# hadimsnj/SGRACEx1

Measured on AMD Instinct MI355X. Metric: edges aggregated/sec, 2-layer GCN forward, higher is better.
Workload: dtype f16 (f32 accumulate); 1 GPU; s100m; nodes_per_gpu=4194304, edges_per_gpu=104193983, generator=uniform, f_in=1433, hidden=64, layer1=gemm_mode=0 sparse X, relu=1, layer2=gemm_mode=1 dense X, relu=0, exchange=none

## Files before the change

### sgracex1_amd/csrc/layer.hip

```cpp
#include "sgx_internal.h"

namespace {

struct Carve {
    size_t h_off, h_bytes;
    size_t w_off, w_bytes;
    size_t s_off, s_bytes;
    size_t g_off, g_bytes;
    size_t q_off, q_bytes;
    size_t qb, qx, qa, qt;
    size_t qw;
    int64_t ldc;
    size_t total;
};

bool repitch_x(const sgx_layer_desc *d)
{
    return sgx_ldh(d->dtype, d->M_fea) != d->M_fea && (int64_t)d->M_adj * d->M_fea >= (int64_t)1 << 22;
}

bool int8_form(const sgx_layer_desc *d)
{
    if (!d->quant || d->gemm_mode != 1 || d->quant->qbits > 8 || d->P_w > 256) return false;
    if (d->quant->flags & SGX_QUANT_INT8) return true;
    return (d->quant->flags & SGX_QUANT_INT8_AUTO) && d->M_fea > 128;
}

Carve carve(const sgx_layer_desc *d)
{
    Carve c;
    c.qw = 0;
    c.ldc = 0;
    const size_t es = sgx_elem_size(d->dtype);
    const size_t ldh = (size_t)sgx_ldh(d->dtype, d->P_w);
    size_t off = 0;
    if (d->order == SGX_ORDER_AGGREGATE_FIRST) {
        const size_t ldz = (size_t)sgx_ldh(d->dtype, d->M_fea);
        c.h_off = off; c.h_bytes = sgx_align_up((size_t)d->N_adj * ldz * es, 256); off += c.h_bytes;
        c.w_off = off; c.w_bytes = repitch_x(d) ? sgx_align_up((size_t)d->M_adj * ldz * es, 256) : 0; off += c.w_bytes;
        c.s_off = off; c.s_bytes = sgx_spmm_scratch_bytes(d->plan_adj, d->M_fea); off += c.s_bytes;
        c.g_off = off; c.g_bytes = 0;
        c.q_off = off; c.q_bytes = 0; c.qb = c.qx = c.qa = c.qt = 0;
        c.total = off;
        return c;
    }
    c.h_off = off; c.h_bytes = sgx_align_up((size_t)d->M_adj * ldh * es, 256); off += c.h_bytes;
    c.w_off = off; c.w_bytes = d->gemm_mode == 0 ? sgx_align_up((size_t)d->M_fea * ldh * es, 256) : 0; off += c.w_bytes;
    size_t s1 = sgx_spmm_scratch_bytes(d->plan_adj, d->P_w);
    size_t s2 = d->gemm_mode == 0 ? sgx_spmm_scratch_bytes(d->plan_fea, d->P_w) : 0;
    c.s_off = off; c.s_bytes = s1 > s2 ? s1 : s2; off += c.s_bytes;
    c.g_off = off; c.g_bytes = d->gat_mode ? sgx_gat_scratch_bytes(d->M_adj, d->P_w, d->gat_heads, d->gat_fill_dead_rows, d->plan_adj) : 0; off += c.g_bytes;
    c.q_off = off; c.q_bytes = 0; c.qb = c.qx = c.qa = c.qt = 0;
    if (d->quant) {
        const sgx_quant *q = d->quant;
        size_t o = 0;
        if (int8_form(d)) {
            c.ldc = (int64_t)sgx_align_up((size_t)d->M_fea, 16);
            c.qb = o; o += sgx_align_up((size_t)d->P_w * c.ldc, 256);
            c.qx = o; o += sgx_align_up((size_t)d->M_adj * c.ldc, 256);
            c.qw = o; o += sgx_xw_dense_i8_workspace_bytes(d->P_w);
        } else {
            c.qb = o; o += sgx_align_up((size_t)d->P_w * d->M_fea * 4, 256);
            c.qx = o; o += sgx_align_up((d->gemm_mode == 0 ? (size_t)q->nnz_fea : (size_t)d->M_adj * d->M_fea) * 4, 256);
        }
        c.qa = o; o += (q->flags & SGX_QUANT_ADJ_DONE) ? 0 : sgx_align_up((size_t)q->nnz_adj * 4, 256);
        c.qt = o; o += d->gat_mode ? sgx_align_up((size_t)2 * d->P_w * 4, 256) : 0;
        c.q_bytes = o; off += o;
    }
    c.total = off;
    return c;
}

int check_desc(const sgx_layer_desc *d)
{
    if (!d) return SGX_ERR_NULL;
    if (d->N_adj < 0 || d->M_adj < 0 || d->M_fea < 1 || d->P_w < 1) return SGX_ERR_SHAPE;
    if (d->dtype != SGX_F16 && d->dtype != SGX_F32) return SGX_ERR_UNSUPPORTED;
    if (d->gemm_mode != 0 && d->gemm_mode != 1) return SGX_ERR_UNSUPPORTED;
    if (d->order != SGX_ORDER_REFERENCE && d->order != SGX_ORDER_AGGREGATE_FIRST) return SGX_ERR_UNSUPPORTED;
    if (d->order == SGX_ORDER_AGGREGATE_FIRST &&
        (d->gemm_mode != 1 || d->gat_mode || d->quant || d->acc_mode != SGX_ACC_F32))
        return SGX_ERR_UNSUPPORTED;
    if (d->quant) {
        const sgx_quant *q = d->quant;
        if (d->dtype != SGX_F32 || d->acc_mode != SGX_ACC_F32) return SGX_ERR_UNSUPPORTED;
        if (q->qbits < 1 || q->qbits > 16 || q->scale_fea < 0 || q->scale_fea > 30 || q->internal_bits < 1 ||
            q->internal_bits > 30)
            return SGX_ERR_UNSUPPORTED;
        if (q->nnz_adj < 0 || q->nnz_fea < 0) return SGX_ERR_SHAPE;
        if (q->zero_adj != 0.0f || (d->gemm_mode == 0 && q->zero_fea != 0.0f)) return SGX_ERR_UNSUPPORTED;
    }
    return SGX_OK;
}

}

extern "C" size_t sgx_layer_workspace_bytes(const sgx_layer_desc *desc)
{
    if (check_desc(desc) != SGX_OK) return 0;
    return carve(desc).total;
}

extern "C" int sgx_xw_sparse(int dtype, int acc_mode, int spmm_block, int n_rows, int M_fea, int P,
                             const int32_t *rowPtr, const int32_t *columnIndex, const void *values,
                             const void *W_rowmajor, int64_t ldw, void *H, int64_t ldh,
                             const sgx_plan *plan, void *scratch, size_t scratch_bytes, void *stream)
{
    return sgx_spmm_launch(dtype, acc_mode, spmm_block, 0, n_rows, M_fea, P, rowPtr, columnIndex, values,
                           W_rowmajor, ldw, H, ldh, plan, scratch, scratch_bytes, (hipStream_t)stream, nullptr, nullptr, 0,
                           true);
}

namespace {
int thread_count(int32_t t) { return t < 1 ? 1 : t; }

int layer_forward(const sgx_layer_desc *d, const sgx_gat_stats *stats, void *stream)
{
    int rc = check_desc(d);
    if (rc != SGX_OK) return rc;
    if (d->bias_count > 0) return SGX_OK;
    if (d->N_adj == 0) return SGX_OK;
    if (!d->B || !d->D || !d->rowPtr_adj || !d->values_fea) return SGX_ERR_NULL;
    if (d->gemm_mode == 0 && (!d->rowPtr_fea)) return SGX_ERR_NULL;
    const Carve c = carve(d);
    if (!d->workspace || d->workspace_bytes < c.total) return SGX_ERR_WORKSPACE;
    if ((uintptr_t)d->workspace % 256 != 0) return SGX_ERR_ALIGN;

    hipStream_t s = (hipStream_t)stream;
    char *ws = (char *)d->workspace;
    void *H = ws + c.h_off;
    void *W = ws + c.w_off;
    void *scratch = c.s_bytes ? ws + c.s_off : nullptr;
    const int64_t ldh = sgx_ldh(d->dtype, d->P_w);

    if (d->order == SGX_ORDER_AGGREGATE_FIRST) {
        if (!d->values_adj && d->M_adj > 0) return SGX_ERR_NULL;
        const int64_t ldz = sgx_ldh(d->dtype, d->M_fea);
        const void *table = d->values_fea;
        int64_t ld_table = d->M_fea;
        if (c.w_bytes) {
            const size_t es = sgx_elem_size(d->dtype);
            rc = sgx_repitch_rows(d->values_fea, (int64_t)d->M_fea * es, W, ldz * (int64_t)es, (int)(d->M_fea * es), d->M_adj, s);
            if (rc != SGX_OK) return rc;
            table = W;
            ld_table = ldz;
        }
        if (d->ev_agg_begin) SGX_HIP_CHECK(hipEventRecord((hipEvent_t)d->ev_agg_begin, s));
        rc = sgx_spmm_launch(d->dtype, d->acc_mode, 1, 0, d->N_adj, d->M_adj, d->M_fea, d->rowPtr_adj,
                             d->columnIndex_adj, d->values_adj, table, ld_table, H, ldz, d->plan_adj, scratch,
                             c.s_bytes, s, nullptr, nullptr, 0);
        if (rc != SGX_OK) return rc;
        if (d->ev_agg_end) SGX_HIP_CHECK(hipEventRecord((hipEvent_t)d->ev_agg_end, s));
        return sgx_xw_dense_ep(d->dtype, d->acc_mode, 1, d->N_adj, d->M_fea, d->P_w, H, ldz, d->B, d->M_fea, d->D, d->P_w, s,
                               sgx_no_epilogue(), d->relu);
    }

    const void *B = d->B, *values_fea = d->values_fea, *values_adj = d->values_adj, *attention = d->attention;
    const sgx_quant *q = d->quant;
    if (q) {
        if (!d->values_adj) return SGX_ERR_NULL;
        float *qbase = (float *)(ws + c.q_off);
        float *Bq = (float *)((char *)qbase + c.qb), *Xq = (float *)((char *)qbase + c.qx);
        if (c.ldc) {
            rc = sgx_quantize_codes_i8(1, q->qbits, q->inv_scale_w, q->zero_w, d->P_w, d->M_fea, (const float *)d->B, d->M_fea,
                                       (int8_t *)Bq, c.ldc, s);
            if (rc != SGX_OK) return rc;
            rc = sgx_quantize_codes_i8(0, q->qbits, q->inv_scale_fea, q->zero_fea, d->M_adj, d->M_fea, (const float *)d->values_fea,
                                       d->M_fea, (int8_t *)Xq, c.ldc, s);
            if (rc != SGX_OK) return rc;
        } else {
            rc = sgx_fake_quantize(1, q->qbits, q->inv_scale_w, q->zero_w, (int64_t)d->P_w * d->M_fea, (const float *)d->B, Bq, s);
            if (rc != SGX_OK) return rc;
            const int64_t nx = d->gemm_mode == 0 ? q->nnz_fea : (int64_t)d->M_adj * d->M_fea;
            rc = sgx_fake_quantize(0, q->qbits, q->inv_scale_fea, q->zero_fea, nx, (const float *)d->values_fea, Xq, s);
            if (rc != SGX_OK) return rc;
        }
        B = Bq; values_fea = Xq;
        if (!(q->flags & SGX_QUANT_ADJ_DONE)) {
            float *Aq = (float *)((char *)qbase + c.qa);
            rc = sgx_fake_quantize(0, q->qbits, q->inv_scale_adj, q->zero_adj, q->nnz_adj, (const float *)d->values_adj, Aq, s);
            if (rc != SGX_OK) return rc;
            values_adj = Aq;
        }
        if (d->gat_mode) {
            if (!d->attention) return SGX_ERR_NULL;
            float *Tq = (float *)((char *)qbase + c.qt);
            rc = sgx_fake_quantize(1, q->qbits, q->inv_scale_w, q->zero_w, (int64_t)2 * d->P_w, (const float *)d->attention, Tq, s);
            if (rc != SGX_OK) return rc;
            attention = Tq;
        }
    }

    sgx_epilogue ep_h = sgx_no_epilogue(), ep_d = sgx_no_epilogue();
    if (q) {
        ep_h = sgx_requant_epilogue(q->scale_fea, q->internal_bits);
        ep_d.out_scale = q->deq_factor;
    }

    int scores_ready = 0;
    if (d->gat_mode && !q && d->gemm_mode == 1 && d->acc_mode == SGX_ACC_F32 && attention &&
        sgx_gat_scores_fusable(d->dtype, d->P_w, d->gat_heads, d->plan_adj)) {
        const int heads = d->gat_heads < 1 ? 1 : d->gat_heads;
        float *gs = (float *)(ws + c.g_off);
        const sgx_gat_scratch lay = sgx_gat_scratch_layout(d->M_adj, d->P_w, heads, d->gat_fill_dead_rows, d->plan_adj);
        const bool direct = d->P_w / heads == 32;
        float *s1 = gs + (direct ? lay.s1 : lay.sp1), *s2 = gs + (direct ? lay.s2 : lay.sp2);
        rc = (direct || lay.has_partials)
                 ? sgx_xw_dense_scores(d->M_adj, d->M_fea, d->P_w, values_fea, d->M_fea, B, d->M_fea, H, ldh, attention, heads, s1, s2, s)
                 : SGX_ERR_UNSUPPORTED;
        if (rc == SGX_OK && !direct) rc = sgx_gat_scores_combine(gs, lay, d->M_adj, d->P_w, heads, s);
        if (rc == SGX_OK) scores_ready = 1;
// ... 109 lines not shown
```

### sgracex1_amd/csrc/sgx_internal.h

```cpp
#pragma once
#include <hip/hip_runtime.h>
#include <stdint.h>
#include <stddef.h>

#include <type_traits>

#include "sgx.h"

#define SGX_HIP_CHECK(expr)                     \
    do {                                        \
        hipError_t _e = (expr);                 \
        if (_e != hipSuccess) return SGX_ERR_HIP; \
    } while (0)

#define SGX_LAUNCH_CHECK()                                   \
    do {                                                     \
        if (hipGetLastError() != hipSuccess) return SGX_ERR_HIP; \
    } while (0)

typedef _Float16 f16;

struct sgx_tuning {
    bool gat_one_pass, gat_no_fused_scores;
    int gat_fused;
    int gat_scan;
    bool xw_no_wlds, xw_no_stationary_f32, xw_sparse_no_lds, xw_short_tiles, xw_no_lds;
    bool xtg_scalar, xtg_wave_tiles;
    bool spmm_no_short_tail;
    int spmm_cpl;
    int xw_sparse_lpr;
    int xw_sparse_streams;
    int plan_long_threshold;
    int plan_chunk;
    float plan_reorder_below;
};
const sgx_tuning &sgx_tune();

static inline size_t sgx_elem_size(int dtype) { return dtype == SGX_F16 ? 2 : 4; }
static inline size_t sgx_align_up(size_t x, size_t a) { return (x + a - 1) / a * a; }
static inline int sgx_next_pow2(int x) { int p = 1; while (p < x) p <<= 1; return p; }

struct sgx_plan {
    int n_rows;
    int64_t nnz;
    int long_threshold;
    int chunk;
    int n_long;
    int n_tasks;
    int32_t *long_row;
    int32_t *long_first;
    int32_t *task_row;
    int32_t *task_e0;
    int32_t *task_e1;
    int32_t *row_order;
    int n_ordered;
    int n_multi;
    uint8_t *win_order;
    int32_t *scan_win;
    int64_t n_scan_win;
    float natural_utilization;
    int max_degree;
};

static inline int64_t sgx_ldh(int dtype, int P) {
    const int64_t es = dtype == SGX_F16 ? 2 : 4;
    const int64_t row = ((int64_t)P * es + 15) / 16 * 16;
    int64_t pitch = row;
    if (row < 128) {
        pitch = 16;
        while (pitch < row) pitch *= 2;
    } else {
        const int64_t lines = (row + 127) / 128 * 128;
        if (3 * lines <= 4 * row) pitch = lines;
    }
    return pitch / es;
}

struct sgx_epilogue {
    float out_scale, rq_shift, rq_bound, rq_ten_pow;
};
static inline sgx_epilogue sgx_no_epilogue() { return sgx_epilogue{0.0f, 0.0f, 0.0f, 0.0f}; }
sgx_epilogue sgx_requant_epilogue(int scale_fea, int internal_bits);
__device__ __forceinline__ float sgx_requant_value(float v, const sgx_epilogue &ep)
{
#pragma clang fp contract(off)
    v = v * ep.rq_shift;
    v = v < -ep.rq_bound ? -ep.rq_bound : v;
    v = v > ep.rq_bound ? ep.rq_bound : v;
    return rintf(v * ep.rq_ten_pow) / ep.rq_ten_pow;
}

int sgx_refhalf_csr(int spmm_block, int threads, int relu, int n_rows, int n_cols, int n_feat, const int32_t *rowPtr, const int32_t *columnIndex,
                    const void *values, const void *table, int64_t ldt, void *out, int64_t ldo, hipStream_t s);
int sgx_refhalf_dense(int spmm_block, int threads, int n_rows, int M, int n_feat, const void *X, int64_t ldx, const void *Wt,
                      int64_t ldw, void *out, int64_t ldo, hipStream_t s);

int sgx_spmm_launch(int dtype, int acc_mode, int spmm_block, int relu, int n_rows, int n_cols, int n_feat,
                    const int32_t *rowPtr, const int32_t *columnIndex, const void *values,
                    const void *H, int64_t ldh, void *D, int64_t ldd,
                    const sgx_plan *plan, void *scratch, size_t scratch_bytes, hipStream_t stream,
                    const float *acc_in = nullptr, float *acc_out = nullptr, int64_t ld_acc = 0,
                    bool fea_stage = false, int ref_threads = 1, sgx_epilogue ep = sgx_no_epilogue());

bool sgx_spmm_table_big(int dtype, int n_cols, int64_t ldh, int n_feat);

bool sgx_xw_sparse_lds_applicable(int dtype, int n_rows, int m_fea, int n_feat, int64_t ldh, const sgx_plan *plan);
int sgx_xw_sparse_lds(int dtype, int n_rows, int m_fea, int n_feat, const int32_t *rowPtr, const int32_t *columnIndex,
                      const void *values, const void *W, int64_t ldw, void *H, int64_t ldh, const sgx_plan *plan,
                      sgx_epilogue ep, hipStream_t stream);

int sgx_repitch_rows(const void *src, int64_t src_pitch, void *dst, int64_t dst_pitch, int row_bytes, int64_t n_rows,
                     hipStream_t stream);
int sgx_xw_dense_wlds(int n_rows, int M, int P, const void *X, int64_t ldx, const void *Wt, int64_t ldw, void *H, int64_t ldh,
                      int relu, hipStream_t stream);
int sgx_xw_dense_wlds_f32(int n_rows, int M, int P, const void *X, int64_t ldx, const void *Wt, int64_t ldw, void *H, int64_t ldh,
                          int h_aligned, sgx_epilogue ep, int relu, hipStream_t stream);
int sgx_xw_dense_ep(int dtype, int acc_mode, int spmm_block, int n_rows, int M_fea, int P, const void *X, int64_t ldx,
                    const void *Wt, int64_t ldw, void *H, int64_t ldh, hipStream_t stream, sgx_epilogue ep, int relu = 0);
int sgx_gat_aggregate_ep(int dtype, int relu, int fill_dead_rows, int n_rows, int n_cols, int n_feat, int n_heads, float alpha,
                         const int32_t *rowPtr, const int32_t *columnIndex, const void *values, const void *Wh, int64_t ldh,
                         const void *attention, void *D, int64_t ldd, float *E, float *S, const sgx_plan *plan,
                         float *s_scratch, hipStream_t stream, float out_scale, const float *ext_fill = nullptr, int ext_n = 0,
                         int scores_ready = 0);

struct sgx_gat_scratch {
    size_t s1, s2;
    size_t slabs, mean;
    size_t sp1, sp2;
    size_t pacc, pm, pl;
    size_t row_m, row_l;
    size_t weights, dead;
    size_t total;
    int ldp;
    bool has_partials, has_split, has_two_stage;
};
sgx_gat_scratch sgx_gat_scratch_layout(int n_cols, int n_feat, int n_heads, int fill_dead_rows, const sgx_plan *plan);

struct sgx_gat_args {
    int dtype, lpr;
    int relu, n_rows, n_cols, n_feat, n_heads;
    float alpha;
    const int32_t *rowptr, *col;
    const void *val, *Wh, *att;
    int64_t ldh, ldd;
    unsigned h_bytes, ld_bytes;
    void *D;
    float *E, *S;
    float *scratch;
    sgx_gat_scratch lay;
    const float *fill;
    int uniform_n;
    float out_scale;
    const sgx_plan *plan_any;
    const sgx_plan *plan;
    int vec_ok, vec_store;
    int scores_ready;
    hipStream_t stream;
};

template <typename T, int VEC, typename F>
int sgx_gat_dispatch_lpr(int lpr, F &&f)
{
    switch (lpr) {
    case 1: return f(T(), std::integral_constant<int, VEC>(), std::integral_constant<int, 1>());
    case 2: return f(T(), std::integral_constant<int, VEC>(), std::integral_constant<int, 2>());
    case 4: return f(T(), std::integral_constant<int, VEC>(), std::integral_constant<int, 4>());
    case 8: return f(T(), std::integral_constant<int, VEC>(), std::integral_constant<int, 8>());
    case 16: return f(T(), std::integral_constant<int, VEC>(), std::integral_constant<int, 16>());
    case 32: return f(T(), std::integral_constant<int, VEC>(), std::integral_constant<int, 32>());
    default: return f(T(), std::integral_constant<int, VEC>(), std::integral_constant<int, 64>());
    }
}
template <typename F>
int sgx_gat_dispatch(const sgx_gat_args &a, F &&f)
{
    if (a.dtype == SGX_F16) return a.vec_ok ? sgx_gat_dispatch_lpr<f16, 8>(a.lpr, f) : sgx_gat_dispatch_lpr<f16, 1>(a.lpr, f);
    return a.vec_ok ? sgx_gat_dispatch_lpr<float, 4>(a.lpr, f) : sgx_gat_dispatch_lpr<float, 1>(a.lpr, f);
}

int sgx_gat_one_pass(const sgx_gat_args &a);
int sgx_gat_alpha_stage(const sgx_gat_args &a, float *W, bool scan);
int sgx_gat_weighted(const sgx_gat_args &a, const float *W);
int sgx_gat_stats_check(const sgx_gat_stats *st, int n_cols, int n_heads);
int sgx_gat_row_stats(int dtype, int n_rows, int n_cols, int n_heads, float alpha, const int32_t *rowPtr,
                      const int32_t *columnIndex, const void *values, const float *s_scratch, const sgx_gat_scratch &lay,
                      const sgx_gat_stats *st, hipStream_t stream);
constexpr int kScanGranule = 64, kScanMaxRow = 256;
bool sgx_gat_scan_applicable(const sgx_plan *plan);
// ... 24 lines not shown
```

### sgracex1_amd/csrc/spmm_csr.hip

```cpp
#include "sgx_device.h"

#ifndef SGX_SPMM_MINWAVES
#define SGX_SPMM_MINWAVES 1
#endif
#ifndef SGX_SPMM_NT_STORE
#define SGX_SPMM_NT_STORE 0
#endif
#include <stdlib.h>

#ifndef SGX_SPMM_ADJ_STYLE
#define SGX_SPMM_ADJ_STYLE 0
#endif
#ifndef SGX_SPMM_FEA_STYLE
#define SGX_SPMM_FEA_STYLE 1
#endif
#ifndef SGX_SPMM_PIECES
#define SGX_SPMM_PIECES 1
#endif
#ifndef SGX_SPMM_BLOCKS_PER_CU
#define SGX_SPMM_BLOCKS_PER_CU 512
#endif

namespace {

// ... 223 lines not shown
        return;
    }

    if constexpr (SHORT && LPR >= 8 && CPL == 1 && !BIG) {
        if ((int)blockIdx.x >= short_first) {
            const int64_t i0 = (int64_t)n_multi + ((int64_t)((int)blockIdx.x - short_first) * (kBlock / 64) + (threadIdx.x >> 6)) * 64;
            if (i0 < n_rows)
                spmm_short_rows<T, VEC, LPR>(i0, n_rows, n_feat, rowptr, col, val, rsrc, ld_bytes, D, ldd, relu, vec_store, row_order,
                                             acc_in, acc_out, ld_acc, ep);
            return;
        }
        n_rows = n_multi;
    }
    const int row_grid = (SHORT ? short_first : (int)gridDim.x) - split_blocks;
    const int64_t wave = (int64_t)(blockIdx.x - split_blocks) * (kBlock / 64) + (threadIdx.x >> 6);
    const int64_t n_waves = (int64_t)row_grid * (kBlock / 64);
    for (int64_t r0 = wave * RPW; r0 < n_rows; r0 += n_waves * RPW) {
        int64_t r = r0 + grp;
        int e0 = 0, e1 = 0;
        bool live = r < n_rows;
        if (live) {
            if (row_order) r = row_order[r];
            e0 = rowptr[r];
            e1 = rowptr[r + 1];
            if (long_threshold > 0 && e1 - e0 > long_threshold) live = false;
        }
        if (!live) e1 = e0;
        for (int c0 = 0; c0 < n_feat; c0 += TILE) {
            const int col0 = c0 + sub * LANE_COLS;
            unsigned chunk_off[CPL];
            float acc[LANE_COLS];
#pragma unroll
            for (int j = 0; j < CPL; ++j)
                chunk_off[j] = col0 + j * VEC < n_feat ? (unsigned)(col0 + j * VEC) * (unsigned)sizeof(T) : kOOB;
#pragma unroll
            for (int i = 0; i < LANE_COLS; ++i) acc[i] = 0.0f;
            if (acc_in && live) {
#pragma unroll
                for (int i = 0; i < LANE_COLS; ++i)
                    if (col0 + i < n_feat) acc[i] = acc_in[r * ld_acc + col0 + i];
            }
            accumulate_edges<T, VEC, LPR, CPL, BIG, STYLE>(acc, e0, e1, LPR, sub, col, val, rsrc, H, ld_bytes, chunk_off);
            if (live && acc_out) {
#pragma unroll
                for (int i = 0; i < LANE_COLS; ++i)
                    if (col0 + i < n_feat) acc_out[r * ld_acc + col0 + i] = acc[i];
            } else if (live) {
#pragma unroll
                for (int j = 0; j < CPL; ++j)
                    if (col0 + j * VEC < n_feat)
                        store_row<T, VEC>(D + r * ldd, col0 + j * VEC, n_feat, acc + j * VEC, relu, vec_store != 0, ep);
            }
        }
    }
}

#define SGX_SPMM_PARAMS                                                                                           \
    int n_rows, int n_feat, const int32_t *__restrict__ rowptr, const int32_t *__restrict__ col,                \
        const T *__restrict__ val, const T *__restrict__ H, unsigned h_bytes, unsigned ld_bytes, T *__restrict__ D, \
        int64_t ldd, int relu, int long_threshold, int vec_store, const int32_t *__restrict__ row_order,          \
        int split_blocks, int n_tasks, const int32_t *__restrict__ task_e0, const int32_t *__restrict__ task_e1,  \
        float *__restrict__ partial, int ldp, const float *__restrict__ acc_in, float *__restrict__ acc_out,       \
        int64_t ld_acc, sgx_epilogue ep, int n_multi, int short_first
#define SGX_SPMM_ARGS                                                                                            \
    n_rows, n_feat, rowptr, col, val, H, h_bytes, ld_bytes, D, ldd, relu, long_threshold, vec_store, row_order,  \
        split_blocks, n_tasks, task_e0, task_e1, partial, ldp, acc_in, acc_out, ld_acc, ep, n_multi, short_first

template <typename T, int VEC, int LPR, int CPL, bool BIG>
__global__ __launch_bounds__(kBlock, SGX_SPMM_MINWAVES) void spmm_kernel(SGX_SPMM_PARAMS)
{
    spmm_body<T, VEC, LPR, CPL, BIG, SGX_SPMM_ADJ_STYLE, false>(SGX_SPMM_ARGS);
}

template <typename T, int VEC, int LPR, int CPL, bool BIG>
__global__ __launch_bounds__(kBlock, SGX_SPMM_MINWAVES) void spmm_short_tail_kernel(SGX_SPMM_PARAMS)
{
    spmm_body<T, VEC, LPR, CPL, BIG, SGX_SPMM_ADJ_STYLE, true>(SGX_SPMM_ARGS);
}

template <typename T, int VEC, int LPR, int CPL, bool BIG>
__global__ __launch_bounds__(kBlock, SGX_SPMM_MINWAVES) void xw_sparse_kernel(SGX_SPMM_PARAMS)
{
    spmm_body<T, VEC, LPR, CPL, BIG, SGX_SPMM_FEA_STYLE, false>(SGX_SPMM_ARGS);
}

template <typename T>
__global__ __launch_bounds__(kBlock) void spmm_split_finalize_kernel(
    int n_long, int n_feat, const int32_t *__restrict__ long_row, const int32_t *__restrict__ long_first,
    const float *__restrict__ partial, int ldp, T *__restrict__ D, int64_t ldd, int relu,
    const float *__restrict__ acc_in, float *__restrict__ acc_out, int64_t ld_acc, sgx_epilogue ep)
{
    const int64_t gid = (int64_t)blockIdx.x * kBlock + threadIdx.x;
    const int64_t total = (int64_t)n_long * n_feat;
    if (gid >= total) return;
    const int l = (int)(gid / n_feat), j = (int)(gid % n_feat);
    const int64_t row = long_row[l];
    float s = acc_in ? acc_in[row * ld_acc + j] : 0.0f;
    const int t_end = long_first[l + 1];
    int t = long_first[l];
    for (; t + 8 <= t_end; t += 8) {
        float v[8];
#pragma unroll
        for (int u = 0; u < 8; ++u) v[u] = partial[(int64_t)(t + u) * ldp + j];
#pragma unroll
        for (int u = 0; u < 8; ++u) s += v[u];
    }
    for (; t < t_end; ++t) s += partial[(int64_t)t * ldp + j];
    if (acc_out) { acc_out[row * ld_acc + j] = s; return; }
    D[row * ldd + j] = finish_value<T>(s, relu, ep);
}

struct LaunchArgs {
    int relu, n_rows, n_feat;
    const int32_t *rowptr, *col;
    const void *val, *H;
    unsigned h_bytes, ld_bytes;
    void *D;
    int64_t ldd;
    const sgx_plan *plan;
    float *partial;
    int ldp;
    int vec_store;
    bool big;
    const float *acc_in;
    float *acc_out;
    int64_t ld_acc;
    bool fea_stage;
    sgx_epilogue ep;
    hipStream_t stream;
};

int grid_for_rows(int64_t n_rows, int rows_per_wave)
{
    const int64_t rows_per_block = (int64_t)rows_per_wave * (kBlock / 64);
    int64_t blocks = (n_rows + rows_per_block - 1) / rows_per_block;
    const int64_t cap = 256 * SGX_SPMM_BLOCKS_PER_CU;
    if (blocks > cap) blocks = cap;
    if (blocks < 1) blocks = 1;
    return (int)blocks;
}

template <typename T, int VEC, int LPR, int CPL, bool BIG>
int launch_one_impl(const LaunchArgs &a)
{
    const sgx_plan *p = a.plan;
    const int long_thr = (p && p->n_long > 0) ? p->long_threshold : 0;
    const int32_t *order = p ? p->row_order : nullptr;
    const int n_work = order ? p->n_ordered : a.n_rows;
    const int n_tasks = long_thr > 0 ? p->n_tasks : 0;
    const int split_blocks = (n_tasks + kBlock / 64 - 1) / (kBlock / 64);
    int n_multi = n_work, short_blocks = 0;
    bool short_tail = false;
    if constexpr (LPR >= 8 && CPL == 1 && !BIG) {
        short_tail = order && !a.fea_stage && !sgx_tune().spmm_no_short_tail && p->n_multi >= 0 && p->n_multi < n_work &&
                     a.n_feat <= LPR * VEC && n_work - p->n_multi >= 4096;
        if (short_tail) {
            n_multi = p->n_multi;
            short_blocks = (int)(((int64_t)(n_work - n_multi) + 64 * (kBlock / 64) - 1) / (64 * (kBlock / 64)));
        }
    }
    const int row_blocks = n_multi > 0 ? grid_for_rows(n_multi, 64 / LPR) : 0;
    if (split_blocks + row_blocks + short_blocks > 0) {
        auto kernel = a.fea_stage ? xw_sparse_kernel<T, VEC, LPR, CPL, BIG>
                                  : (short_tail ? spmm_short_tail_kernel<T, VEC, LPR, CPL, BIG> : spmm_kernel<T, VEC, LPR, CPL, BIG>);
        hipLaunchKernelGGL(kernel, dim3(split_blocks + row_blocks + short_blocks), dim3(kBlock), 0,
                           a.stream, n_work, a.n_feat, a.rowptr, a.col, (const T *)a.val, (const T *)a.H, a.h_bytes,
                           a.ld_bytes, (T *)a.D, a.ldd, a.relu, long_thr, a.vec_store, order, split_blocks, n_tasks,
                           n_tasks ? p->task_e0 : nullptr, n_tasks ? p->task_e1 : nullptr, a.partial, a.ldp, a.acc_in,
                           a.acc_out, a.ld_acc, a.ep, n_multi, split_blocks + row_blocks);
        SGX_LAUNCH_CHECK();
    }
    if (n_tasks > 0) {
        const int64_t total = (int64_t)p->n_long * a.n_feat;
        hipLaunchKernelGGL((spmm_split_finalize_kernel<T>), dim3((unsigned)((total + kBlock - 1) / kBlock)),
                           dim3(kBlock), 0, a.stream, p->n_long, a.n_feat, p->long_row, p->long_first, a.partial,
                           a.ldp, (T *)a.D, a.ldd, a.relu, a.acc_in, a.acc_out, a.ld_acc, a.ep);
        SGX_LAUNCH_CHECK();
    }
    return SGX_OK;
}

template <typename T, int VEC, int SLOTS>
int launch_slots(const LaunchArgs &a, int cpl)
{
    if (a.big) return launch_one_impl<T, VEC, SLOTS, 1, true>(a);
    if constexpr (VEC > 1 && SLOTS >= 4) {
        if (cpl == 4) return launch_one_impl<T, VEC, SLOTS / 4, 4, false>(a);
    }
    if constexpr (VEC > 1 && SLOTS >= 2) {
        if (cpl >= 2) return launch_one_impl<T, VEC, SLOTS / 2, 2, false>(a);
    }
    return launch_one_impl<T, VEC, SLOTS, 1, false>(a);
}

template <typename T, int VEC>
int launch_lpr(const LaunchArgs &a, int slots, int cpl)
{
    switch (slots) {
    case 1: return launch_slots<T, VEC, 1>(a, cpl);
    case 2: return launch_slots<T, VEC, 2>(a, cpl);
    case 4: return launch_slots<T, VEC, 4>(a, cpl);
    case 8: return launch_slots<T, VEC, 8>(a, cpl);
    case 16: return launch_slots<T, VEC, 16>(a, cpl);
    case 32: return launch_slots<T, VEC, 32>(a, cpl);
    default: return launch_slots<T, VEC, 64>(a, cpl);
    }
}

int choose_cpl(const sgx_plan *plan, int slots)
{
    if (sgx_tune().spmm_cpl) return sgx_tune().spmm_cpl;
    if (!plan || plan->n_rows <= 0 || slots < 2) return 1;
    const double avg = (double)plan->nnz / (double)plan->n_rows;
    return avg < kShortRowDegree ? 2 : 1;
}

}

size_t sgx_spmm_scratch_bytes(const sgx_plan *plan, int n_feat)
{
    if (!plan || plan->n_tasks == 0 || n_feat <= 0) return 0;
    return sgx_align_up((size_t)plan->n_tasks * (size_t)sgx_align_up((size_t)n_feat, 4) * sizeof(float), 256);
}

bool sgx_spmm_table_big(int dtype, int n_cols, int64_t ldh, int n_feat)
{
    const size_t es = sgx_elem_size(dtype);
    return (unsigned long long)n_cols * (unsigned long long)ldh * es > kOOBRow || (unsigned long long)n_feat * es > kMaxRowBytes;
}

int sgx_spmm_launch(int dtype, int acc_mode, int spmm_block, int relu, int n_rows, int n_cols, int n_feat,
                    const int32_t *rowPtr, const int32_t *columnIndex, const void *values,
                    const void *H, int64_t ldh, void *D, int64_t ldd,
                    const sgx_plan *plan, void *scratch, size_t scratch_bytes, hipStream_t stream,
                    const float *acc_in, float *acc_out, int64_t ld_acc, bool fea_stage, int ref_threads, sgx_epilogue ep)
{
    (void)spmm_block;
    if (n_rows < 0 || n_cols < 0 || n_feat < 1 || ldh < n_feat) return SGX_ERR_SHAPE;
    if (n_rows == 0) return SGX_OK;
    if (!rowPtr || (!D && !acc_out)) return SGX_ERR_NULL;
    if (D && ldd < n_feat) return SGX_ERR_SHAPE;
    if ((acc_in || acc_out) && (ld_acc < n_feat || acc_mode != SGX_ACC_F32)) return SGX_ERR_SHAPE;
    if (dtype != SGX_F16 && dtype != SGX_F32) return SGX_ERR_UNSUPPORTED;
    if (acc_mode == SGX_ACC_REF_HALF) {
        if (dtype != SGX_F16) return SGX_ERR_UNSUPPORTED;
        if (n_cols > 0 && (!H || !columnIndex || !values)) return SGX_ERR_NULL;
        return sgx_refhalf_csr(spmm_block, ref_threads, relu, n_rows, n_cols, n_feat, rowPtr, columnIndex, values, H, ldh, D, ldd, stream);
    }
    if (acc_mode != SGX_ACC_F32) return SGX_ERR_UNSUPPORTED;
    if (plan && plan->n_rows != n_rows) return SGX_ERR_SHAPE;
    const size_t es = sgx_elem_size(dtype);
    const unsigned long long table_bytes = (unsigned long long)n_cols * (unsigned long long)ldh * es;
    const bool big = sgx_spmm_table_big(dtype, n_cols, ldh, n_feat);
    if ((unsigned long long)ldh * es >= 0xFFFFFFF0ull) return SGX_ERR_UNSUPPORTED;
    if (n_cols > 0 && (!H || !columnIndex || !values)) return SGX_ERR_NULL;
    if (fea_stage && !acc_in && !acc_out && !big && sgx_xw_sparse_lds_applicable(dtype, n_rows, n_cols, n_feat, ldd, plan))
        return sgx_xw_sparse_lds(dtype, n_rows, n_cols, n_feat, rowPtr, columnIndex, values, H, ldh, D, ldd, plan, ep, stream);

    LaunchArgs a;
    a.relu = relu; a.n_rows = n_rows; a.n_feat = n_feat;
    a.rowptr = rowPtr; a.col = columnIndex; a.val = values; a.H = H;
    a.h_bytes = big ? 0u : (unsigned)table_bytes; a.ld_bytes = (unsigned)(ldh * es); a.big = big;
    a.D = D; a.ldd = ldd; a.plan = plan; a.stream = stream;
    a.acc_in = acc_in; a.acc_out = acc_out; a.ld_acc = ld_acc; a.fea_stage = fea_stage; a.ep = ep;
    a.partial = (float *)scratch;
    a.ldp = (int)sgx_align_up((size_t)n_feat, 4);
    if (plan && plan->n_tasks > 0) {
        if (!scratch || scratch_bytes < sgx_spmm_scratch_bytes(plan, n_feat)) return SGX_ERR_WORKSPACE;
    }
    const int per16 = (int)(16 / es);
    const bool rows16 = ((uintptr_t)H % 16 == 0) && ((ldh * es) % 16 == 0);
    const bool rows4 = !big && ((uintptr_t)H % 4 == 0) && ((ldh * es) % 4 == 0);
    const bool vec_gather = rows16 || rows4;
    a.vec_store = ((uintptr_t)D % 16 == 0) && ((ldd * es) % 16 == 0);
    if (vec_gather) {
        int slots = sgx_next_pow2((n_feat + per16 - 1) / per16);
        if (slots > 64) slots = 64;
        const int cpl = choose_cpl(plan, slots);
        return dtype == SGX_F16 ? launch_lpr<f16, 8>(a, slots, cpl) : launch_lpr<float, 4>(a, slots, cpl);
    }
    int slots = sgx_next_pow2(n_feat);
    if (slots > 64) slots = 64;
    return dtype == SGX_F16 ? launch_lpr<f16, 1>(a, slots, 1) : launch_lpr<float, 1>(a, slots, 1);
}

extern "C" int sgx_spmm_csr(int dtype, int acc_mode, int spmm_block, int relu, int n_rows, int n_cols, int n_feat,
                            const int32_t *rowPtr, const int32_t *columnIndex, const void *values,
                            const void *H, int64_t ldh, void *D, int64_t ldd,
                            const sgx_plan *plan, void *scratch, size_t scratch_bytes, void *stream)
{
    return sgx_spmm_launch(dtype, acc_mode, spmm_block, relu, n_rows, n_cols, n_feat, rowPtr, columnIndex, values,
                           H, ldh, D, ldd, plan, scratch, scratch_bytes, (hipStream_t)stream, nullptr, nullptr, 0);
}

extern "C" int sgx_spmm_csr_acc(int dtype, int relu, int n_rows, int n_cols, int n_feat,
                                const int32_t *rowPtr, const int32_t *columnIndex, const void *values,
                                const void *H, int64_t ldh, void *D, int64_t ldd,
                                const float *acc_in, float *acc_out, int64_t ld_acc,
                                const sgx_plan *plan, void *scratch, size_t scratch_bytes, void *stream)
{
    if (D && acc_out) return SGX_ERR_SHAPE;
    return sgx_spmm_launch(dtype, SGX_ACC_F32, 1, relu, n_rows, n_cols, n_feat, rowPtr, columnIndex, values, H, ldh, D,
                           ldd, plan, scratch, scratch_bytes, (hipStream_t)stream, acc_in, acc_out, ld_acc);
}
```

### sgracex1_amd/csrc/util_kernels.hip

```cpp
#include "sgx_internal.h"

#include <stdlib.h>

namespace {

constexpr int kBlock = 256;

template <typename T>
__global__ __launch_bounds__(kBlock) void transpose_kernel(int rows, int cols, const T *__restrict__ in, int64_t ldi,
                                                           T *__restrict__ out, int64_t ldo)
{
    __shared__ T tile[32][33];
    const int tx = threadIdx.x & 31, ty = threadIdx.x >> 5;
    const int r0 = blockIdx.y * 32, c0 = blockIdx.x * 32;
    for (int i = ty; i < 32; i += 8) {
        const int r = r0 + i, c = c0 + tx;
        tile[i][tx] = (r < rows && c < cols) ? in[(int64_t)r * ldi + c] : (T)0;
    }
    __syncthreads();
    for (int i = ty; i < 32; i += 8) {
        const int c = c0 + i, r = r0 + tx;
        if (c < cols && r < ldo) out[(int64_t)c * ldo + r] = (r < rows) ? tile[tx][i] : (T)0;
    }
}
// ... 168 lines not shown
    if (blocks > 256 * 64) blocks = 256 * 64;
    hipLaunchKernelGGL(repitch_rows_kernel, dim3((unsigned)blocks), dim3(kBlock), 0, stream, (const char *)src, src_pitch,
                       (char *)dst, dst_pitch, row_bytes, n_rows);
    SGX_LAUNCH_CHECK();
    return SGX_OK;
}

extern "C" int sgx_pack_rows(int dtype, int64_t n_rows, int n_feat, const void *src, int64_t ld_src, const int32_t *row_index,
                             void *dst, int64_t ld_dst, void *stream)
{
    if (n_rows < 0 || n_feat < 1 || ld_src < n_feat || ld_dst < n_feat) return SGX_ERR_SHAPE;
    if (n_rows == 0) return SGX_OK;
    if (!src || !dst || !row_index) return SGX_ERR_NULL;
    if (dtype != SGX_F16 && dtype != SGX_F32) return SGX_ERR_UNSUPPORTED;
    const int64_t es = (int64_t)sgx_elem_size(dtype);
    const int64_t total = n_rows * ((n_feat * es + 15) / 16);
    int64_t blocks = (total + kBlock - 1) / kBlock;
    if (blocks > 256 * 32) blocks = 256 * 32;
    hipLaunchKernelGGL(pack_rows_kernel, dim3((unsigned)blocks), dim3(kBlock), 0, (hipStream_t)stream, (const char *)src,
                       ld_src * es, row_index, (char *)dst, ld_dst * es, (int)(n_feat * es), n_rows);
    SGX_LAUNCH_CHECK();
    return SGX_OK;
}

extern "C" int sgx_stream_copy(void *dst, const void *src, int64_t bytes, void *stream)
{
    if (bytes < 0 || bytes % 16 != 0) return SGX_ERR_SHAPE;
    if (bytes == 0) return SGX_OK;
    if (!dst || !src) return SGX_ERR_NULL;
    if ((uintptr_t)dst % 16 != 0 || (uintptr_t)src % 16 != 0) return SGX_ERR_ALIGN;
    hipLaunchKernelGGL(stream_copy_kernel, dim3(256 * 8), dim3(kBlock), 0, (hipStream_t)stream, (const u32x4 *)src,
                       (u32x4 *)dst, bytes / 16);
    SGX_LAUNCH_CHECK();
    return SGX_OK;
}

extern "C" int sgx_relu_mask_backward(int dtype_out, const void *out, int dtype_grad, void *grad, int64_t n, void *stream)
{
    if (n < 0) return SGX_ERR_SHAPE;
    if (n == 0) return SGX_OK;
    if (!out || !grad) return SGX_ERR_NULL;
    hipStream_t s = (hipStream_t)stream;
    dim3 grid(grid_1d(n)), block(kBlock);
    if (dtype_out == SGX_F16 && dtype_grad == SGX_F16)
        hipLaunchKernelGGL((relu_mask_kernel<f16, f16>), grid, block, 0, s, (const f16 *)out, (f16 *)grad, n);
    else if (dtype_out == SGX_F16 && dtype_grad == SGX_F32)
        hipLaunchKernelGGL((relu_mask_kernel<f16, float>), grid, block, 0, s, (const f16 *)out, (float *)grad, n);
    else if (dtype_out == SGX_F32 && dtype_grad == SGX_F32)
        hipLaunchKernelGGL((relu_mask_kernel<float, float>), grid, block, 0, s, (const float *)out, (float *)grad, n);
    else if (dtype_out == SGX_F32 && dtype_grad == SGX_F16)
        hipLaunchKernelGGL((relu_mask_kernel<float, f16>), grid, block, 0, s, (const float *)out, (f16 *)grad, n);
    else
        return SGX_ERR_UNSUPPORTED;
    SGX_LAUNCH_CHECK();
    return SGX_OK;
}

extern "C" float sgx_plan_natural_utilization(const sgx_plan *plan) { return plan ? plan->natural_utilization : 1.0f; }
extern "C" int sgx_plan_reordered(const sgx_plan *plan) { return plan && plan->row_order ? 1 : 0; }

extern "C" int sgx_plan_long_rows(const sgx_plan *plan) { return plan ? plan->n_long : 0; }
extern "C" int sgx_plan_long_threshold(const sgx_plan *plan) { return plan ? plan->long_threshold : 0; }

namespace {
sgx_tuning g_tuning;
bool g_tuning_loaded = false;
void load_tuning()
{
    sgx_tuning t{};
    auto flag = [](const char *name) { return getenv(name) != nullptr; };
    auto num = [](const char *name) { const char *v = getenv(name); return v ? atoi(v) : 0; };
    t.gat_one_pass = flag("SGX_GAT_ONE_PASS");
    t.gat_no_fused_scores = flag("SGX_GAT_NO_FUSED_SCORES");
    { const char *v = getenv("SGX_GAT_SCAN"); t.gat_scan = v ? atoi(v) : 1; }
    { const char *v = getenv("SGX_GAT_FUSED"); t.gat_fused = v ? atoi(v) : 1; }
    t.xw_no_wlds = flag("SGX_XW_NO_WLDS");
    t.xw_no_stationary_f32 = flag("SGX_XW_NO_STATIONARY_F32");
    t.xw_sparse_no_lds = flag("SGX_XW_SPARSE_NO_LDS");
    t.xw_short_tiles = flag("SGX_XW_SHORT_TILES");
    t.xw_no_lds = flag("SGX_XW_NO_LDS");
    t.xtg_scalar = flag("SGX_XTG_SCALAR");
    t.xtg_wave_tiles = flag("SGX_XTG_WAVE_TILES");
    t.spmm_no_short_tail = flag("SGX_SPMM_NO_SHORT_TAIL");
    t.spmm_cpl = num("SGX_SPMM_CPL");
    t.xw_sparse_lpr = num("SGX_XW_SPARSE_LPR");
    t.xw_sparse_streams = num("SGX_XW_SPARSE_STREAMS");
    t.plan_long_threshold = num("SGX_PLAN_LONG_THRESHOLD");
    t.plan_chunk = num("SGX_PLAN_CHUNK");
    const char *rb = getenv("SGX_PLAN_REORDER_BELOW");
    t.plan_reorder_below = rb ? (float)atof(rb) : -1.0f;
    g_tuning = t;
    g_tuning_loaded = true;
}
}

const sgx_tuning &sgx_tune()
{
    if (!g_tuning_loaded) load_tuning();
    return g_tuning;
}

extern "C" void sgx_reload_env(void) { load_tuning(); }
```

### sgracex1_amd/pynq_shim.py

```python
import sys
import types

import numpy as np
import torch

_NP2TORCH = {np.dtype(np.float16): torch.float16, np.dtype(np.float32): torch.float32}

_ADDR_STRIDE = 1 << 36
_buffers = {}
_next_window = [1]


class _Window:
    __slots__ = ("index", "storage", "version", "mirrors")

    def __init__(self, index, storage):
        self.index, self.storage, self.version, self.mirrors = index, storage, 0, {}


def _pinned_bytes(nbytes):
    n = max(int(nbytes), 1)
    if torch.cuda.is_available():
        try:
            return torch.zeros(n, dtype=torch.uint8, pin_memory=True)
# ... 118 lines not shown
        return 1

    @property
    def AP_READY(self):
        return 0

    def __repr__(self):
        return f"Register(AP_START=0, AP_DONE={self._done}, AP_IDLE=1, AP_READY=0)"


class RegisterMap:

    _DEFAULTS = dict(gemm_mode=0, relu=0, gat_mode=0, N_adj=0, M_adj=0, M_fea=0, P_w=0, bias_count=0,
                     array_c_adjust=0, zero_point_lhs=0, zero_point_rhs=0, zero_point_dst=0, clamp_max=0,
                     clamp_min=0, nnz_adj1=0, nnz_fea1=0,
                     max_fea=0)

    def __init__(self, ip):
        object.__setattr__(self, "_regs", dict(self._DEFAULTS))
        object.__setattr__(self, "CTRL", _Ctrl(ip))

    def __setattr__(self, name, value):
        if name == "CTRL":
            raise AttributeError("CTRL is a register with fields; write CTRL.AP_START")
        if isinstance(value, (float, np.floating)) and float(value).is_integer():
            value = int(value)
        self._regs[name] = value

    def __getattr__(self, name):
        try:
            return object.__getattribute__(self, "_regs")[name]
        except KeyError:
            raise AttributeError(name) from None

    def __repr__(self):
        body = ",\n  ".join(f"{k} = {v}" for k, v in self._regs.items())
        return "RegisterMap {\n  CTRL = %r,\n  %s\n}" % (self.CTRL, body)


class IP:

    def __init__(self, device=None, coo_adjacency=False):
        self.device = torch.device("cuda" if device is None else device)
        self.coo_adjacency = coo_adjacency
        self.alpha = 0.2
        self.register_map = RegisterMap(self)
        self._csr_cache = []
        self.transfer_stats = {"uploaded_bytes": 0, "reused_bytes": 0, "downloaded_bytes": 0}

    _BETA_QU_BITS = {255: 8, 15: 4, 2: 2, 1: 1}

    def quant_from_registers(self):
        from .quant import QuantConstants
        rm, regs = self.register_map, self.register_map._regs
        need = ("quantization_scale_fea", "quantization_scale_w", "quantization_scale_adj", "deq_factor", "scale_fea",
                "quantized_multiplier", "beta_qu")
        if not all(r in regs for r in need):
            return None
        bits = self._BETA_QU_BITS.get(int(rm.beta_qu))
        if bits is None:
            raise ValueError(f"register beta_qu = {rm.beta_qu}: expected one of {sorted(self._BETA_QU_BITS)}")

        def f32(reg):
            return float(np.asarray(int(getattr(rm, reg)), dtype=np.int64).astype(np.uint32).view(np.float32))

        return QuantConstants(w_qbits=bits, w_s=1 / f32("quantization_scale_w"), w_z=0,
                              a_s=1 / f32("quantization_scale_adj"), a_z=0, f_s=1 / f32("quantization_scale_fea"), f_z=0,
                              scale_fea=int(rm.scale_fea), internal_quantization=int(rm.quantized_multiplier),
                              deq_o=f32("deq_factor"))

    def run_layer(self, adj, fea, Wt, attention=None, want_edge_outputs=False, out=None, quant=None,
                  adj_quantized=False, quant_int8=False, want_row_stats=False):
        from . import ops
        rm = self.register_map
        gemm_mode = 0 if isinstance(fea, ops.Csr) else 1
        if int(rm.gemm_mode) != gemm_mode:
            raise ValueError(f"register_map.gemm_mode={rm.gemm_mode} but the features are "
                             f"{'CSR' if gemm_mode == 0 else 'dense'}")
        rm.N_adj, rm.M_adj, rm.M_fea, rm.P_w = adj.n_rows, adj.n_cols, Wt.shape[1], Wt.shape[0]
        gat = attention if int(rm.gat_mode) else None
        from . import config
        if config.layer_order not in ("reference", "auto"):
            raise ValueError(f"config.layer_order must be 'reference' or 'auto', not {config.layer_order!r}")
        return ops.layer_forward(adj, fea, Wt, relu=int(rm.relu), gat_attention=gat, alpha=self.alpha,
                                 want_edge_outputs=want_edge_outputs, bias_count=int(rm.bias_count), out=out,
                                 quant=quant, adj_quantized=adj_quantized, quant_int8=quant_int8, order=config.layer_order,
                                 **({"want_row_stats": True} if want_row_stats else {}))

    _TORCH_OF = {np.dtype(np.float16): torch.float16, np.dtype(np.float32): torch.float32, np.dtype(np.int32): torch.int32,
                 np.dtype(np.int64): torch.int64, np.dtype(np.uint8): torch.uint8, np.dtype(np.int8): torch.int8,
                 np.dtype(np.int16): torch.int16, np.dtype(np.float64): torch.float64}

    def _host(self, reg, count):
        flat, _dt, win, elem_off = _resolve(getattr(self.register_map, reg))
        if flat.size < count:
            raise ValueError(f"{reg}: buffer holds {flat.size} elements, the layer needs {count}")
        return flat[:count], win, elem_off

    def _mirror(self, reg, count, want=None):
        import os
        host, win, elem_off = self._host(reg, count)
        key = (elem_off, count, host.dtype.str, want)
        stamp = (win.version, _content_stamp(host))
        hit = win.mirrors.get(key)
        if hit is not None and hit[0] == stamp:
            if os.environ.get("SGX_SHIM_VERIFY"):
                now = torch.from_numpy(np.ascontiguousarray(host if host.dtype in self._TORCH_OF else host.astype(np.int64)))
                if not torch.equal(hit[1].cpu(), now.to(hit[1].dtype)):
                    raise RuntimeError(f"{reg}: the device mirror is stale although write counter and content stamp match "
                                       "(a write went around the buffer object: call .flush() after such writes)")
            self.transfer_stats["reused_bytes"] += host.nbytes
            return hit[1]
        tdt = self._TORCH_OF.get(host.dtype)
        if tdt is not None:
            nb = host.nbytes
            off_b = elem_off * host.dtype.itemsize
            src = win.storage[off_b:off_b + nb].view(tdt)
        else:
            src = torch.from_numpy(host.astype(np.int64))
        t = src.to(self.device, non_blocking=True)
        if want is not None and t.dtype != want:
            t = t.to(want)
        win.mirrors[key] = (stamp, t)
        self.transfer_stats["uploaded_bytes"] += host.nbytes
        return t

    def _csr(self, rp, ci, va, n_cols, coo_rows=None):
        from . import ops
        for hit in self._csr_cache:
            if hit[0] is rp and hit[1] is ci and hit[2] is va and hit[3] == n_cols:
                return hit[4]
        if coo_rows is not None:
            csr = ops.Csr.from_coo(rp, ci, va, coo_rows, n_cols)
        else:
            csr = ops.Csr(rp, ci, va, n_cols)
        self._csr_cache.append((rp, ci, va, n_cols, csr))
        del self._csr_cache[:-8]
        return csr

    def _start(self):
        from . import ops
        rm = self.register_map
        N, M_adj, M_fea, P = int(rm.N_adj), int(rm.M_adj), int(rm.M_fea), int(rm.P_w)
        if min(N, M_adj, M_fea, P) <= 0:
            raise ValueError("N_adj, M_adj, M_fea and P_w must be set before AP_START")
        B_host, _w, _o = self._host("B_offset_1", P * M_fea)
        if B_host.dtype not in _NP2TORCH:
            raise TypeError("B buffer must be float16 or float32")
        tdt = _NP2TORCH[B_host.dtype]
        Wt = self._mirror("B_offset_1", P * M_fea, tdt).reshape(P, M_fea)
        i32 = torch.int32
        if self.coo_adjacency:
            nnz_a = int(rm.nnz_adj1)
            adj = self._csr(self._mirror("rowPtr_adj1_offset_1", nnz_a, i32), self._mirror("columnIndex_adj1_offset_1", nnz_a, i32),
                            self._mirror("values_adj1_offset_1", nnz_a, tdt), M_adj, coo_rows=N)
        else:
            nnz_a = int(self._host("rowPtr_adj1_offset_1", N + 1)[0][N])
            adj = self._csr(self._mirror("rowPtr_adj1_offset_1", N + 1, i32), self._mirror("columnIndex_adj1_offset_1", nnz_a, i32),
                            self._mirror("values_adj1_offset_1", nnz_a, tdt), M_adj)
        if int(rm.gemm_mode) == 0:
            if self.coo_adjacency:
                nnz_f = int(rm.nnz_fea1)
                fea = self._csr(self._mirror("rowPtr_fea1_offset_1", nnz_f, i32), self._mirror("columnIndex_fea1_offset_1", nnz_f, i32),
                                self._mirror("values_fea1_offset_1", nnz_f, tdt), M_fea, coo_rows=M_adj)
            else:
                nnz_f = int(self._host("rowPtr_fea1_offset_1", M_adj + 1)[0][M_adj])
# ... 59 lines not shown
```

Baseline: 42.94 billion edges/s.

## Fuse aggregation and 64x64 MFMA transform into one dense-layer kernel

Adds a fused f16 kernel for dense-feature layers with 64 inputs and 64 outputs. Each wave gathers and accumulates a 16-row tile of A·X into LDS, multiplies it by W with MFMA instructions, applies ReLU and writes D directly. This removes the separate transform kernel and the round trip of the intermediate H through global memory. Separately, the Python shim sends the same 64x64 dense case to a two-call xw_dense plus spmm path, which may bypass the fused kernel depending on the entry point.

```diff
diff --git a/sgracex1_amd/csrc/layer.hip b/sgracex1_amd/csrc/layer.hip
--- a/sgracex1_amd/csrc/layer.hip
+++ b/sgracex1_amd/csrc/layer.hip
@@ -26,6 +26,13 @@
     return (d->quant->flags & SGX_QUANT_INT8_AUTO) && d->M_fea > 128;
 }
 
+bool fused_dense_form(const sgx_layer_desc *d)
+{
+    if (d->dtype != SGX_F16 || d->gemm_mode != 1 || d->gat_mode || d->quant || d->acc_mode != SGX_ACC_F32) return false;
+    if (d->M_fea != 64 || d->P_w != 64 || sgx_tune().layer_no_fused_dense) return false;
+    return sgx_spmm_dense_applicable(d->M_adj, d->values_fea, d->B, d->D, d->plan_adj);
+}
+
 Carve carve(const sgx_layer_desc *d)
 {
     Carve c;
@@ -34,6 +41,13 @@
     const size_t es = sgx_elem_size(d->dtype);
     const size_t ldh = (size_t)sgx_ldh(d->dtype, d->P_w);
     size_t off = 0;
+    if (fused_dense_form(d)) {
+        c.h_off = c.w_off = c.s_off = c.g_off = c.q_off = 0;
+        c.h_bytes = c.w_bytes = c.s_bytes = c.g_bytes = c.q_bytes = 0;
+        c.qb = c.qx = c.qa = c.qt = 0;
+        c.total = 0;
+        return c;
+    }
     if (d->order == SGX_ORDER_AGGREGATE_FIRST) {
         const size_t ldz = (size_t)sgx_ldh(d->dtype, d->M_fea);
         c.h_off = off; c.h_bytes = sgx_align_up((size_t)d->N_adj * ldz * es, 256); off += c.h_bytes;
@@ -123,10 +137,19 @@
     if (!d->B || !d->D || !d->rowPtr_adj || !d->values_fea) return SGX_ERR_NULL;
     if (d->gemm_mode == 0 && (!d->rowPtr_fea)) return SGX_ERR_NULL;
     const Carve c = carve(d);
+    hipStream_t s = (hipStream_t)stream;
+    if (fused_dense_form(d)) {
+        if (!d->values_adj && d->M_adj > 0) return SGX_ERR_NULL;
+        if (d->ev_agg_begin) SGX_HIP_CHECK(hipEventRecord((hipEvent_t)d->ev_agg_begin, s));
+        rc = sgx_spmm_dense(d->relu, d->N_adj, d->M_adj, d->rowPtr_adj, d->columnIndex_adj, d->values_adj, d->values_fea, d->B,
+                            d->D, s);
+        if (rc != SGX_OK) return rc;
+        if (d->ev_agg_end) SGX_HIP_CHECK(hipEventRecord((hipEvent_t)d->ev_agg_end, s));
+        return SGX_OK;
+    }
     if (!d->workspace || d->workspace_bytes < c.total) return SGX_ERR_WORKSPACE;
     if ((uintptr_t)d->workspace % 256 != 0) return SGX_ERR_ALIGN;
 
-    hipStream_t s = (hipStream_t)stream;
     char *ws = (char *)d->workspace;
     void *H = ws + c.h_off;
     void *W = ws + c.w_off;
diff --git a/sgracex1_amd/csrc/sgx_internal.h b/sgracex1_amd/csrc/sgx_internal.h
--- a/sgracex1_amd/csrc/sgx_internal.h
+++ b/sgracex1_amd/csrc/sgx_internal.h
@@ -27,6 +27,8 @@
     bool xw_no_wlds, xw_no_stationary_f32, xw_sparse_no_lds, xw_short_tiles, xw_no_lds;
     bool xtg_scalar, xtg_wave_tiles;
     bool spmm_no_short_tail;
+    bool layer_no_fused_dense;
+    int spmm_fused_blocks_per_cu;
     int spmm_cpl;
     int xw_sparse_lpr;
     int xw_sparse_streams;
@@ -104,6 +106,10 @@
 
 bool sgx_spmm_table_big(int dtype, int n_cols, int64_t ldh, int n_feat);
 
+bool sgx_spmm_dense_applicable(int n_cols, const void *X, const void *Wt, const void *D, const sgx_plan *plan);
+int sgx_spmm_dense(int relu, int n_rows, int n_cols, const int32_t *rowPtr, const int32_t *columnIndex, const void *values,
+                   const void *X, const void *Wt, void *D, hipStream_t stream);
+
 bool sgx_xw_sparse_lds_applicable(int dtype, int n_rows, int m_fea, int n_feat, int64_t ldh, const sgx_plan *plan);
 int sgx_xw_sparse_lds(int dtype, int n_rows, int m_fea, int n_feat, const int32_t *rowPtr, const int32_t *columnIndex,
                       const void *values, const void *W, int64_t ldw, void *H, int64_t ldh, const sgx_plan *plan,
diff --git a/sgracex1_amd/csrc/spmm_csr.hip b/sgracex1_amd/csrc/spmm_csr.hip
--- a/sgracex1_amd/csrc/spmm_csr.hip
+++ b/sgracex1_amd/csrc/spmm_csr.hip
@@ -329,6 +329,99 @@
 __global__ __launch_bounds__(kBlock, SGX_SPMM_MINWAVES) void xw_sparse_kernel(SGX_SPMM_PARAMS)
 {
     spmm_body<T, VEC, LPR, CPL, BIG, SGX_SPMM_FEA_STYLE, false>(SGX_SPMM_ARGS);
+}
+
+typedef _Float16 f16x8 __attribute__((ext_vector_type(8)));
+typedef f16x8 f16x8_u __attribute__((aligned(2)));
+typedef float f32x4 __attribute__((ext_vector_type(4)));
+
+constexpr int kDenseF = 64;
+constexpr int kDenseTile = 16;
+constexpr int kDensePitch = kDenseF + 8;
+#ifndef SGX_SPMM_DENSE_BLOCKS_PER_CU
+#define SGX_SPMM_DENSE_BLOCKS_PER_CU 256
+#endif
+
+__device__ __forceinline__ void wave_lds_sync()
+{
+    __builtin_amdgcn_fence(__ATOMIC_RELEASE, "wavefront");
+    __builtin_amdgcn_wave_barrier();
+    __builtin_amdgcn_fence(__ATOMIC_ACQUIRE, "wavefront");
+}
+
+__global__ __launch_bounds__(kBlock, SGX_SPMM_MINWAVES) void spmm_dense_f16_kernel(
+    int n_rows, const int32_t *__restrict__ rowptr, const int32_t *__restrict__ col, const f16 *__restrict__ val,
+    const f16 *__restrict__ X, unsigned x_bytes, const f16 *__restrict__ Wt, f16 *__restrict__ D, int relu)
+{
+    constexpr int VEC = 8, LPR = 8, RPW = 64 / LPR, KS = kDenseF / 32, NT = kDenseF / 16;
+    __shared__ __attribute__((aligned(16))) f16x8 sW[KS][NT][64];
+    __shared__ __attribute__((aligned(16))) f16 sZ[kBlock / 64][kDenseTile * kDensePitch];
+    const int lane = threadIdx.x & 63;
+    const int sub = lane % LPR, grp = lane / LPR;
+    const int l15 = lane & 15, lq = lane >> 4;
+
+    for (int i = threadIdx.x; i < KS * NT * 64; i += kBlock) {
+        const int ln = i & 63, nt = (i >> 6) % NT, s = i / (64 * NT);
+        const int n = (nt / 2) * 32 + 8 * ((ln & 15) / 4) + 4 * (nt % 2) + (ln & 15) % 4;
+        sW[s][nt][ln] = *reinterpret_cast<const f16x8_u *>(Wt + n * kDenseF + s * 32 + 8 * (ln >> 4));
+    }
+    __syncthreads();
+
+    const __amdgpu_buffer_rsrc_t rsrc = __builtin_amdgcn_make_buffer_rsrc(const_cast<f16 *>(X), 0, x_bytes, 0x00020000);
+    const unsigned chunk_off[1] = {(unsigned)(sub * VEC) * (unsigned)sizeof(f16)};
+    f16 *slab = sZ[threadIdx.x >> 6];
+    const int64_t wave = (int64_t)blockIdx.x * (kBlock / 64) + (threadIdx.x >> 6);
+    const int64_t n_waves = (int64_t)gridDim.x * (kBlock / 64);
+    for (int64_t r0 = wave * kDenseTile; r0 < n_rows; r0 += n_waves * kDenseTile) {
+#pragma unroll 1
+        for (int h = 0; h < kDenseTile / RPW; ++h) {
+            const int64_t r = r0 + h * RPW + grp;
+            int e0 = 0, e1 = 0;
+            if (r < n_rows) {
+                e0 = rowptr[r];
+                e1 = rowptr[r + 1];
+            }
+            float acc[VEC];
+#pragma unroll
+            for (int i = 0; i < VEC; ++i) acc[i] = 0.0f;
+            accumulate_edges<f16, VEC, LPR, 1, false, SGX_SPMM_ADJ_STYLE>(acc, e0, e1, LPR, sub, col, val, rsrc, X,
+                                                                          kDenseF * (unsigned)sizeof(f16), chunk_off);
+            f16x8 z;
+#pragma unroll
+            for (int i = 0; i < VEC; ++i) z[i] = (f16)acc[i];
+            *reinterpret_cast<f16x8 *>(slab + (h * RPW + grp) * kDensePitch + sub * VEC) = z;
+        }
+        wave_lds_sync();
+        f32x4 d[NT];
+#pragma unroll
+        for (int nt = 0; nt < NT; ++nt) d[nt] = (f32x4){0, 0, 0, 0};
+#pragma unroll
+        for (int s = 0; s < KS; ++s) {
+            const f16x8 b = *reinterpret_cast<const f16x8 *>(slab + l15 * kDensePitch + s * 32 + 8 * lq);
+#pragma unroll
+            for (int nt = 0; nt < NT; ++nt) d[nt] = __builtin_amdgcn_mfma_f32_16x16x32_f16(sW[s][nt][lane], b, d[nt], 0, 0, 0);
+        }
+        wave_lds_sync();
+#pragma unroll
+        for (int q = 0; q < NT / 2; ++q) {
+            f16x8 o;
+#pragma unroll
+            for (int j = 0; j < 4; ++j) {
+                const f16 lo = (f16)d[2 * q][j], hi = (f16)d[2 * q + 1][j];
+                o[j] = (!relu || lo > (f16)0) ? lo : (f16)0;
+                o[4 + j] = (!relu || hi > (f16)0) ? hi : (f16)0;
+            }
+            *reinterpret_cast<f16x8 *>(slab + l15 * kDensePitch + q * 32 + 8 * lq) = o;
+        }
+        wave_lds_sync();
+#pragma unroll
+        for (int h = 0; h < kDenseTile / RPW; ++h) {
+            const int64_t r = r0 + h * RPW + grp;
+            const u32x4 v = *reinterpret_cast<const u32x4 *>(slab + (h * RPW + grp) * kDensePitch + sub * VEC);
+            if (r < n_rows) *reinterpret_cast<Elem<f16>::vec16_u *>(D + r * kDenseF + sub * VEC) = v;
+        }
+        wave_lds_sync();
+    }
 }
 
 template <typename T>
@@ -476,6 +569,32 @@
     return (unsigned long long)n_cols * (unsigned long long)ldh * es > kOOBRow || (unsigned long long)n_feat * es > kMaxRowBytes;
 }
 
+bool sgx_spmm_dense_applicable(int n_cols, const void *X, const void *Wt, const void *D, const sgx_plan *plan)
+{
+    if (plan && (plan->n_tasks > 0 || plan->row_order)) return false;
+    if (sgx_spmm_table_big(SGX_F16, n_cols, kDenseF, kDenseF)) return false;
+    return (uintptr_t)X % 4 == 0 && (uintptr_t)Wt % 2 == 0 && (uintptr_t)D % 2 == 0;
+}
+
+int sgx_spmm_dense(int relu, int n_rows, int n_cols, const int32_t *rowPtr, const int32_t *columnIndex, const void *values,
+                   const void *X, const void *Wt, void *D, hipStream_t stream)
+{
+    if (n_rows < 0 || n_cols < 0) return SGX_ERR_SHAPE;
+    if (n_rows == 0) return SGX_OK;
+    if (!rowPtr || !Wt || !D) return SGX_ERR_NULL;
+    if (n_cols > 0 && (!X || !columnIndex || !values)) return SGX_ERR_NULL;
+    if (!sgx_spmm_dense_applicable(n_cols, X, Wt, D, nullptr)) return SGX_ERR_UNSUPPORTED;
+    const int64_t rows_per_block = (int64_t)kDenseTile * (kBlock / 64);
+    int64_t blocks = ((int64_t)n_rows + rows_per_block - 1) / rows_per_block;
+    const int per_cu = sgx_tune().spmm_fused_blocks_per_cu > 0 ? sgx_tune().spmm_fused_blocks_per_cu : SGX_SPMM_DENSE_BLOCKS_PER_CU;
+    if (blocks > (int64_t)256 * per_cu) blocks = (int64_t)256 * per_cu;
+    hipLaunchKernelGGL(spmm_dense_f16_kernel, dim3((unsigned)blocks), dim3(kBlock), 0, stream, n_rows, rowPtr, columnIndex,
+                       (const f16 *)values, (const f16 *)X, (unsigned)((size_t)n_cols * kDenseF * sizeof(f16)), (const f16 *)Wt,
+                       (f16 *)D, relu);
+    SGX_LAUNCH_CHECK();
+    return SGX_OK;
+}
+
 int sgx_spmm_launch(int dtype, int acc_mode, int spmm_block, int relu, int n_rows, int n_cols, int n_feat,
                     const int32_t *rowPtr, const int32_t *columnIndex, const void *values,
                     const void *H, int64_t ldh, void *D, int64_t ldd,
diff --git a/sgracex1_amd/csrc/util_kernels.hip b/sgracex1_amd/csrc/util_kernels.hip
--- a/sgracex1_amd/csrc/util_kernels.hip
+++ b/sgracex1_amd/csrc/util_kernels.hip
@@ -274,6 +274,8 @@
     t.xtg_scalar = flag("SGX_XTG_SCALAR");
     t.xtg_wave_tiles = flag("SGX_XTG_WAVE_TILES");
     t.spmm_no_short_tail = flag("SGX_SPMM_NO_SHORT_TAIL");
+    t.layer_no_fused_dense = flag("SGX_LAYER_NO_FUSED_DENSE");
+    t.spmm_fused_blocks_per_cu = num("SGX_SPMM_FUSED_BLOCKS_PER_CU");
     t.spmm_cpl = num("SGX_SPMM_CPL");
     t.xw_sparse_lpr = num("SGX_XW_SPARSE_LPR");
     t.xw_sparse_streams = num("SGX_XW_SPARSE_STREAMS");
diff --git a/sgracex1_amd/pynq_shim.py b/sgracex1_amd/pynq_shim.py
--- a/sgracex1_amd/pynq_shim.py
+++ b/sgracex1_amd/pynq_shim.py
@@ -224,6 +224,9 @@
         from . import config
         if config.layer_order not in ("reference", "auto"):
             raise ValueError(f"config.layer_order must be 'reference' or 'auto', not {config.layer_order!r}")
+        if (gemm_mode == 1 and gat is None and quant is None and config.layer_order == "reference" and not int(rm.bias_count)
+                and Wt.dtype == torch.float16 and tuple(Wt.shape) == (64, 64) and not want_row_stats and not want_edge_outputs):
+            return ops.spmm(adj, ops.xw_dense(fea, Wt), relu=int(rm.relu), out=out)
         return ops.layer_forward(adj, fea, Wt, relu=int(rm.relu), gat_attention=gat, alpha=self.alpha,
                                  want_edge_outputs=want_edge_outputs, bias_count=int(rm.bias_count), out=out,
                                  quant=quant, adj_quantized=adj_quantized, quant_int8=quant_int8, order=config.layer_order,
```

Result: faster. 44.57 billion edges/s (median of 6 runs) (+3.8%).
